# EDIpack/EDIpack

Hardware: AMD Instinct MI355X
Metric: Lanczos H*v iterations/sec, largest (Nup,Ndw) sector (higher is better)
Workload: dtype f64

## Files before the change

### edipack_amd/csrc/edigpu_apply.hip

```cpp
#include <algorithm>
#include <cmath>
#include <string>

#include "dev_mem.hpp"
#include "host_ib.hpp"
#include "kernels.hpp"

namespace edigpu {

int ensure_workspace(edigpu_sector* s) {
  const int64_t len = s->nloc * (s->is_complex ? 2 : 1);
  if (s->d_vin && s->ws_len == len) return 0;
  dev_free_all(s->d_vin, s->d_vout, s->d_tmp, s->d_partial, s->d_scal);
  const size_t n = (size_t)std::max<int64_t>(std::max(std::max(len, s->blk_len), s->ib ? s->ib->len : 0), 1);
  EDIGPU_HIP(hipMalloc((void**)&s->d_vin, n * sizeof(double)));
  EDIGPU_HIP(hipMalloc((void**)&s->d_vout, n * sizeof(double)));
  EDIGPU_HIP(hipMalloc((void**)&s->d_tmp, n * sizeof(double)));
  if (s->ib && s->ib->ps != s->ib->dim_dw * kIbPanel) {
    EDIGPU_HIP(hipMemset(s->d_vin, 0, n * sizeof(double)));
    EDIGPU_HIP(hipMemset(s->d_vout, 0, n * sizeof(double)));
    EDIGPU_HIP(hipMemset(s->d_tmp, 0, n * sizeof(double)));
  }
  s->partial_cap = std::max<int64_t>(kMaxPartials, 3 * ((s->nloc + 255) / 256) + 64);
  EDIGPU_HIP(hipMalloc((void**)&s->d_partial, (size_t)s->partial_cap * sizeof(double)));
  s->ws_len = len;
  return 0;
}

static int apply_eph_operator(const edigpu_sector* s, const double* v, double* hv, int w, hipStream_t st) {
  if (!s->sub_a) return 0;
  const int64_t n = s->dim_el * w;
  for (int jph = 0; jph <= s->nph; jph++) {
    if (apply_any(s->sub_a, v + jph * n, v + jph * n, s->d_cz, 3, st)) return 1;
    double* up = jph < s->nph ? hv + (jph + 1) * n : nullptr;
    double* dn = jph > 0 ? hv + (jph - 1) * n : nullptr;
    if (launch_eph_scatter(n, s->d_cz, up, sqrt((double)(jph + 1)), dn, sqrt((double)jph), st)) return 1;
  }
  return 0;
}

int apply_any(edigpu_sector* s, const double* v_local, const double* v_full, double* hv,
              int phase, hipStream_t st) {
  if (s->kind == kCmplxNormal) {
    if (phase != 3) {
      set_error("complex normal-mode sectors are single-shard: use the fused product");
      return 1;
    }
    if (s->sub_d) return apply_any(s->sub_d, v_full, v_full, hv, 3, st);
    const int64_t n = s->dim;
    double *xr = s->d_cz, *xi = xr + n, *yr = xi + n, *yi = yr + n, *t1 = yi + n, *t2 = t1 + n;
    if (launch_deinterleave(n, v_full, xr, xi, st)) return 1;
    if (apply_any(s->sub_s, xr, xr, yr, 3, st) || apply_any(s->sub_s, xi, xi, yi, 3, st)) return 1;
    if (s->sub_a && (apply_any(s->sub_a, xi, xi, t1, 3, st) || apply_any(s->sub_a, xr, xr, t2, 3, st))) return 1;
    return launch_combine_interleave(n, yr, yi, s->sub_a ? t1 : nullptr, s->sub_a ? t2 : nullptr, hv, st);
  }
  if (s->kind == kNormal && s->has_phonons()) {
// ... 325 lines not shown
```

### edipack_amd/csrc/edigpu_internal.hpp

```cpp
#pragma once
#include <hip/hip_runtime.h>

#include <cstdint>
#include <cstdio>
#include <functional>
#include <memory>
#include <string>
#include <vector>

#include "../../include/edigpu.h"
#include "host_build.hpp"
#include "switches.hpp"

namespace edigpu {

enum SectorKind : int { kNormal = 0, kFlat = 1, kDirect = 2, kOrbs = 3, kCmplxNormal = 4 };

void set_error(const std::string& msg);
#pragma GCC visibility push(hidden)
bool have_error();
int current_device();
int ensure_device(int* count_out = nullptr);
#pragma GCC visibility pop

// ... 175 lines not shown
  hipStream_t stream = nullptr;
  int64_t dim = 0, nloc = 0, row_first = 0;
  int64_t dim_up = 0, dim_dw = 0, dw_first = 0, dw_count = 0;
  double* d_hd = nullptr;
  edigpu::DevEll up_ell;
  edigpu::DevCsr dw;
  int dw_maxrow = 0;
  edigpu::DevCsr nd;
  int has_nd = 0;
  edigpu::HostCsr h_up, h_dw;
  int rows_per_block = 1;
  int factored = 0;
  int fac_nimp = 0, fac_nterms = 0;
  double* d_eux = nullptr;
  double* d_ed = nullptr;
  uint8_t* d_impd = nullptr;
  double* d_ndcoef = nullptr;
  uint32_t* d_jup = nullptr;
  edigpu_sector* sub_s = nullptr;
  edigpu_sector* sub_a = nullptr;
  edigpu_sector* sub_d = nullptr;
  double* d_cz = nullptr;
  int panel_mode = 0;
  int tile_nchunks = 0, tile_rows = 0;
  int32_t* d_tile_chunks = nullptr;
  int32_t* d_tile_lbeg = nullptr;
  int tile_list_cap = 0;
  int4* d_tl_meta = nullptr;
  int32_t* d_tl_col = nullptr;
  double* d_tl_val = nullptr;
  int tl_has_nd = 0;
  int blk_shift = 0;
  int blk_tail_balance = 1;
  int64_t blk_ps = 0, blk_len = 0;
  int4* d_bl_meta = nullptr;
  int blk_rows = 0;
  int blk_list_cap = 0;
  int32_t* d_bl_lend = nullptr;
  uint32_t* d_bl_ent = nullptr;
  double* d_bl_wtab = nullptr;
  bool lz_blocked = false;
  int64_t lz_len = 0;
  edigpu::IbDev* ib = nullptr;
  int row_split = 1;
  int col_halo = 0;
  uint32_t* d_jdw = nullptr;
  int32_t* d_mx_rowptr = nullptr;
  int32_t* d_mx_col = nullptr;
  double* d_mx_val = nullptr;
  int nph = 0;
  int64_t dim_el = 0;
  double w0_ph = 0.0, a_ph = 0.0;
  double* d_gu = nullptr;
  double* d_gd = nullptr;
  int64_t nd_nnz = 0;
  std::vector<double> h_hd;
  edigpu::HostCsr h_nd;
  bool lazy_export = false;
  edigpu_model model;
  int sec_a = 0, sec_b = 0;
  bool jz = false;
  bool built_by_library = false;
  bool from_model() const { return built_by_library; }
  bool is_normal_family() const { return kind == edigpu::kNormal || kind == edigpu::kCmplxNormal; }
  bool is_flat_family() const { return kind == edigpu::kFlat || kind == edigpu::kDirect; }
  bool has_phonons() const { return nph > 0; }
// ... 80 lines not shown
```

### edipack_amd/csrc/edigpu_setup.hip

```cpp
#include <algorithm>
#include <cstddef>
#include <memory>

#include "dev_mem.hpp"
#include "host_ib.hpp"
#include "host_pack.hpp"
#include "host_sb.hpp"
#include "kernels.hpp"

namespace edigpu {

static const int4* as_int4(const std::vector<HostInt4>& v) {
  static_assert(sizeof(HostInt4) == sizeof(int4) && offsetof(HostInt4, x) == offsetof(int4, x) &&
                    offsetof(HostInt4, y) == offsetof(int4, y) && offsetof(HostInt4, z) == offsetof(int4, z) &&
                    offsetof(HostInt4, w) == offsetof(int4, w),
                "HostInt4 is uploaded as int4");
  return reinterpret_cast<const int4*>(v.data());
}

static int upload_csr(DevCsr& d, int64_t nrow, const int64_t* rowptr, const int32_t* col,
                      const double* val, int cplx) {
  d = DevCsr();
  d.nrow = nrow;
  d.nnz = rowptr ? rowptr[nrow] : 0;
// ... 423 lines not shown
  if (s->factored && built && built->norb > 0 && dw_first == 0 && dw_count == dim_dw) {
    const int64_t min_rows = sw.ib_min;
    bool pairs = false;
    for (int sp = 0; sp < 2 && !pairs; sp++) {
      const std::vector<double>& a = built->ob_a[sp];
      const int ns = built->ns;
      if ((int)a.size() == ns * ns)
        for (int p = built->norb; p < ns && !pairs; p++)
          for (int q = p + 1; q < ns; q++)
            if (a[(size_t)p * ns + q] != 0.0) {
              pairs = true;
              break;
            }
    }
    const bool pairs_ok = !pairs || min_rows == 0 || sw.ib_pairs;
    const bool short_rows = dim_up * 8 < sw.ib_min_row_bytes();
    if (sw.ib && pairs_ok && s->nloc >= min_rows && (!short_rows || sw.posrows) && !sw.lanczos_unfused && setup_ib(s, *built))
      return 1;
    if (s->ib && short_rows && !s->ib->pr.on) {
      free_ib(s->ib);
      delete s->ib;
      s->ib = nullptr;
    }
  }
  if (!s->ib && s->factored && built && dw_first == 0 && dw_count == dim_dw && s->rows_per_block >= 1 && s->row_split == 1 &&
      dim_dw <= 65535 && dim_up >= 64) {
    const bool on = sw.blocked;
    const int64_t min_rows = sw.blocked_min;
    const int shift = sw.blocked_shift();
    const HostFactored& f = built->fac;
    if (on && shift == 7 && s->nloc >= min_rows && s->panel_mode == 2 && (f.nterms == 0 || s->tl_has_nd)) {
      s->blk_shift = 7;
      s->blk_tail_balance = sw.tile_balance;
      s->blk_rows = s->tile_rows;
      s->blk_ps = dim_dw << 7;
      s->blk_len = ((dim_up + 127) >> 7) * s->blk_ps;
    } else if (on && shift && shift < 7 && s->nloc >= min_rows && f.nterms <= 16) {
      const HostBlockLists b = build_block_lists(dw, f, dim_dw, shift, sw.blocked_lds_kb);
      if (b.fits) {
        s->blk_list_cap = b.list_cap;
        if (dev_upload(&s->d_bl_lend, b.lend.data(), b.lend.size()) || dev_upload(&s->d_bl_meta, as_int4(b.meta), b.meta.size()) ||
            dev_upload(&s->d_bl_ent, b.ent.data(), b.ent.size()) || dev_upload(&s->d_bl_wtab, b.wtab.data(), b.wtab.size()))
          return 1;
        s->blk_shift = shift;
        s->blk_rows = b.rows;
        s->blk_ps = dim_dw << shift;
        s->blk_len = ((dim_up + ((int64_t)1 << shift) - 1) >> shift) * s->blk_ps;
      }
    }
  }
  return finish_handle(s);
}

int setup_flat(edigpu_sector* s, int64_t nrow_local, int64_t ncol_global, int64_t row_first,
               const int64_t* rowptr, const int32_t* col, const double* val, int cplx) {
  s->kind = kFlat;
  s->is_complex = cplx;
  s->device = current_device();
  s->dim = ncol_global;
  s->nloc = nrow_local;
  s->row_first = row_first;
  const int w = cplx ? 2 : 1;
  const int64_t lo = row_first, hi = row_first + nrow_local;
  std::vector<int64_t> rpl((size_t)nrow_local + 1, 0), rpn((size_t)nrow_local + 1, 0);
  for (int64_t i = 0; i < nrow_local; i++) {
    int64_t nl = 0;
// ... 199 lines not shown
```

### edipack_amd/csrc/hooks/image_hooks.hip

```cpp
#include <algorithm>
#include <climits>

#include "../dev_mem.hpp"
#include "../host_pack.hpp"
#include "../kernels.hpp"
#include "../tile_map.hpp"

using namespace edigpu;

extern "C" {

int edigpu_tile_task_map(int32_t npanels, int32_t blocks_per_panel, int32_t balanced, int32_t* grid, int32_t* np,
                         int32_t* panel, int32_t* chunk, int32_t* pos) {
  if (npanels < 1 || blocks_per_panel < 1 || !grid || !np ||
      ((int64_t)npanels + 7) / 8 * 8 * (int64_t)blocks_per_panel > INT32_MAX) {
    set_error("edigpu_tile_task_map: bad argument");
    return 1;
  }
  const TileMap m = plan_tile_map(npanels, blocks_per_panel, balanced != 0);
  *grid = m.grid;
  *np = m.np;
  for (int wg = 0; wg < m.grid; wg++) {
    int pn, ch, ps;
    if (!tile_task_of(m, npanels, blocks_per_panel, wg, pn, ch, ps)) pn = -1;
    if (panel) panel[wg] = pn;
    if (chunk) chunk[wg] = ch;
    if (pos) pos[wg] = ps;
  }
  return 0;
}

int edigpu_ell16_images(int64_t nrow, const int64_t* rowptr, const int32_t* col, const double* val, int64_t* info,
                        uint32_t* pk16, uint32_t* pk16o, int64_t* owned_col) {
  if (nrow < 1 || !rowptr || !info || (rowptr[nrow] > 0 && (!col || !val))) {
    set_error("edigpu_ell16_images: bad argument");
    return 1;
  }
  HostCsr a;
  a.nrow = a.ncol = nrow;
  a.rowptr.assign(rowptr, rowptr + nrow + 1);
  a.col.assign(col, col + rowptr[nrow]);
  a.val.assign(val, val + rowptr[nrow]);
  const HostEll h = encode_ell(a, true, true, true);
  info[0] = h.width;
  info[1] = h.pitch;
  info[2] = h.pitch16o;
  info[3] = (int64_t)h.pk16.size();
  info[4] = (int64_t)h.pk16o.size();
  if (pk16) std::copy(h.pk16.begin(), h.pk16.end(), pk16);
  if (pk16o) std::copy(h.pk16o.begin(), h.pk16o.end(), pk16o);
  if (owned_col)
    for (int64_t pos = 0; pos < h.pitch16o; pos++) owned_col[pos] = ell16_owned_col(pos);
// ... 30 lines not shown
```

### edipack_amd/csrc/kernels_normal.hip

```cpp
#include <cstdlib>
#include <string>
#include <type_traits>

#include "kernels.hpp"
#include "normal_args.hpp"

namespace edigpu {



constexpr int kE = 4;

template <bool VEC>
__device__ inline void load4(const double* __restrict__ base, int64_t i0, const bool* ok, double* out, int64_t dB = 2) {
  if (VEC) {
    const double2 a = ok[0] ? *reinterpret_cast<const double2*>(base + i0) : make_double2(0.0, 0.0);
    const double2 b = ok[2] ? *reinterpret_cast<const double2*>(base + i0 + dB) : make_double2(0.0, 0.0);
    out[0] = a.x;
    out[1] = a.y;
    out[2] = b.x;
    out[3] = b.y;
  } else {
#pragma unroll
    for (int e = 0; e < kE; e++) out[e] = ok[e] ? base[i0 + e] : 0.0;
// ... 520 lines not shown
  a.ell_coef = s->up_ell.coef;
  a.ell_col = s->up_ell.col;
  a.ell_val = s->up_ell.val;
  a.ell_w = s->up_ell.width;
  a.ell_typed = s->up_ell.typed;
  a.ell_pitch = s->up_ell.pitch;
  a.ell_pitch16 = s->up_ell.pitch16;
  a.dw_rowptr = s->dw.rowptr32;
  a.dw_col = s->dw.col;
  a.dw_val = s->dw.val;
  a.dw_maxrow = s->dw_maxrow;
  a.nd_rp32 = s->nd.rowptr32;
  a.nd_rp64 = s->nd.wide ? s->nd.rowptr64 : nullptr;
  a.nd_col = s->nd.col;
  a.nd_val = s->nd.val;
  a.has_nd = s->has_nd;
  a.nterms = s->factored ? s->fac_nterms : 0;
  a.nd_coef = s->d_ndcoef;
  a.jup = s->d_jup;
  a.jdw = s->d_jdw;
  a.panel_mode = s->panel_mode;
  a.tile_nchunks = s->tile_nchunks;
  a.tile_rows = s->tile_rows;
  a.tile_chunks = s->d_tile_chunks;
  a.tile_lbeg = s->d_tile_lbeg;
  a.tile_list_cap = s->tile_list_cap;
  a.tl_meta = s->d_tl_meta;
  a.tl_col = s->d_tl_col;
  a.tl_val = s->d_tl_val;
  a.tl_has_nd = s->tl_has_nd;
  a.blk_shift = 0;
  a.blk_ps = 0;
  a.blk_tail_balance = s->blk_tail_balance;
  a.bl_meta = s->d_bl_meta;
  a.blk_rows = s->blk_rows;
  a.blk_list_cap = s->blk_list_cap;
  a.bl_lend = s->d_bl_lend;
  a.bl_ent = s->d_bl_ent;
  a.bl_wtab = s->d_bl_wtab;
  a.mx_rowptr = s->d_mx_rowptr;
  a.mx_col = s->d_mx_col;
  a.mx_val = s->d_mx_val;
  a.scal = nullptr;
  a.partial = nullptr;
  a.xout = nullptr;
  a.partial_cap = 0;
  a.lz_counter = nullptr;
  a.lz_nlanc = 0;
  a.lz_len = 0;
  a.split_first = 0;
  a.split_count = s->dim_up;
}

int launch_normal(const edigpu_sector* s, const double* v_local, const double* v_full, double* hv,
                  int phase, hipStream_t st) {
  NormalArgs a;
  fill_args(s, a);
  if (s->dw_count == 0) return 0;
  const bool fac = s->factored != 0;
  const bool sell_nd = !fac && s->has_nd && s->nd.sell;
  const bool csr_nd = !fac && s->has_nd && !sell_nd;
  const bool fac_nd = fac && a.nterms > 0 && s->d_mx_rowptr != nullptr;
  if (phase == 1) return launch_rows(s, a, v_local, v_full, hv, 1, st);
  if (phase == 3) {
    if (launch_rows(s, a, v_local, v_full, hv, csr_nd ? 5 : 1, st)) return 1;
    if (launch_dw_panels(a, s->sw, true, fac_nd, v_full, hv, st)) return 1;
// ... 128 lines not shown
```

### edipack_amd/csrc/kernels_panel.hip

```cpp
#include <algorithm>
#include <cstdio>
#include <cstdlib>
#include <vector>

#include "lz_finalize.hpp"
#include "normal_args.hpp"
#include "tile_map.hpp"

namespace edigpu {

struct PanelArgs {
  int npanels, width, blocks_per_panel, rows_per_block;
  int64_t col_first, ncol, stride;
  int halo;
  int tile_rows;
  int list_cap;
  TileMap map;
};

constexpr int kPanelNT = 512;
constexpr int kMaxNdTerms = 16;

template <bool DO_DW, bool DO_ND, bool ALPHA, bool COLS = false>
__global__ void __launch_bounds__(kPanelNT)
// ... 307 lines not shown
      qsum += __shfl_down(qsum, off, 64);
      nsum += __shfl_down(nsum, off, 64);
    }
    if (lane == 0) {
      red[wave] = asum;
      red[kPanelNT / 64 + wave] = qsum;
      red[2 * (kPanelNT / 64) + wave] = nsum;
    }
    __syncthreads();
    double t = 0.0, q = 0.0, n = 0.0;
    if (threadIdx.x == 0) {
#pragma unroll
      for (int i = 0; i < kPanelNT / 64; i++) {
        t += red[i];
        q += red[kPanelNT / 64 + i];
        n += red[2 * (kPanelNT / 64) + i];
      }
      if (!a.lz_counter) {
        a.partial[blockIdx.x] = t;
        a.partial[gridDim.x + blockIdx.x] = q;
        a.partial[2 * gridDim.x + blockIdx.x] = n;
      }
    }
    if (a.lz_counter)
      lz_finalize_if_last<kPanelNT>(a.lz_counter, a.partial, t, q, n, v_full, hv, a.lz_len, const_cast<double*>(a.scal),
                                    a.lz_nlanc, lzsh);
  }
}

constexpr int kTileSeg = 64;
constexpr int kTileRowsPerWave = 4;
constexpr int kTileMaxRows = kTileRowsPerWave * 16;
constexpr int kTileBatch = 4;

template <int NT, bool DO_ND, bool ALPHA, bool EDGE, bool BLK = false>
__global__ void __launch_bounds__(NT)
    normal_dw_tile_kernel(NormalArgs a, PanelArgs p, const double* __restrict__ v_full, double* __restrict__ hv) {
  __shared__ double red[3 * (NT / 64)];
  extern __shared__ double2 tile[];
  double* lval = reinterpret_cast<double*>(tile + (size_t)p.tile_rows * kTileSeg);
  int32_t* lcol = reinterpret_cast<int32_t*>(lval + p.list_cap);
  int4* lmeta = reinterpret_cast<int4*>(lcol + p.list_cap);
  uint32_t* ju2 = reinterpret_cast<uint32_t*>(lmeta + p.tile_rows);
  const int x = blockIdx.x & 7, slot = blockIdx.x >> 3, nslots = gridDim.x >> 3;
  int bpanel = 0, bchunk = 0, ppos = blockIdx.x;
  const int np = BLK ? p.map.np : (int)gridDim.x;
  const bool has_task = !BLK || tile_task_of(p.map, p.npanels, p.blocks_per_panel, blockIdx.x, bpanel, bchunk, ppos);
  if (ALPHA && BLK && (int)blockIdx.x >= p.map.wg_tail && bpanel == p.map.panel_tail && threadIdx.x < 24) {
    const int xx = threadIdx.x & 7;
    if (p.map.panel_tail + xx >= p.npanels) a.partial[(threadIdx.x >> 3) * np + ppos + xx] = 0.0;
  }
  if (ALPHA && a.scal[SC_STOP] != 0.0) {
    if (threadIdx.x == 0) {
      a.partial[ppos] = 0.0;
      a.partial[np + ppos] = 0.0;
      a.partial[2 * np + ppos] = 0.0;
    }
    return;
  }
  double asum = 0.0, qsum = 0.0, nsum = 0.0;
  const double sg = ALPHA ? a.scal[SC_ALPHA] : 0.0;
  const int lane = threadIdx.x & 63;
  const int wave = __builtin_amdgcn_readfirstlane(threadIdx.x >> 6);
  constexpr int NW = NT / 64;
  const int64_t DimUp = a.dim_up;
  int cur_panel = -1;
  for (int task = slot, it = 0;; task += nslots, it++) {
    if (BLK && (it > 0 || !has_task)) break;
    const int panel = BLK ? bpanel : (task / p.blocks_per_panel) * 8 + x;
    if (panel >= p.npanels) break;
    const int chunk = BLK ? bchunk : task % p.blocks_per_panel;
    const int rb = a.tile_chunks[chunk], nrows = a.tile_chunks[chunk + 1] - rb;
    const int lb = a.tile_lbeg[chunk], ln = a.tile_lbeg[chunk + 1] - lb;
    const int64_t pbase = (int64_t)panel * p.width;
    const int64_t RS = BLK ? 128 : DimUp;
    const double* __restrict__ vb = BLK ? v_full + (int64_t)panel * a.blk_ps : v_full;
    double* __restrict__ hb = BLK ? hv + (int64_t)panel * a.blk_ps : hv;
    auto col_of = [&](int l, bool& okl, bool& pairl) -> int64_t {
      const int64_t cl = pbase + 2 * l;
      okl = 2 * l < p.width && cl < DimUp;
      const int64_t ccl = okl ? cl : (EDGE ? DimUp - 1 : DimUp - 2);
      pairl = !EDGE || ccl + 1 < DimUp;
      return ccl;
    };
    bool ok, pair;
    int64_t cc = col_of(lane, ok, pair);
    int64_t c = pbase + 2 * lane;
    if (BLK) {
      cc = c = 2 * lane;
      ok = pair = true;
    }
    auto ld2 = [&](const double* q) -> double2 {
      if (!EDGE) return *reinterpret_cast<const double2*>(q);
      if (pair) {
        const d2u t = *reinterpret_cast<const d2u*>(q);
        return make_double2(t.x, t.y);
      }
      return make_double2(q[0], 0.0);
    };
    auto st2 = [&](double* q, double2 t) {
      if (!EDGE) {
        *reinterpret_cast<double2*>(q) = t;
      } else if (pair) {
        d2u u;
        u.x = t.x;
        u.y = t.y;
        *reinterpret_cast<d2u*>(q) = u;
      } else {
        q[0] = t.x;
      }
    };
    const int64_t g0 = a.dw_first + rb;
    double2 acc[kTileRowsPerWave];
    {
      double2 own[kTileRowsPerWave];
#pragma unroll
      for (int j = 0; j < kTileRowsPerWave; j++) {
        const int r = wave + j * NW;
        const int rr = r < nrows ? r : nrows - 1;
        acc[j] = ld2(&hb[(int64_t)(rb + rr) * RS + cc]);
      }
#pragma unroll
      for (int j = 0; j < kTileRowsPerWave; j++) {
        const int r = wave + j * NW;
        const int rr = r < nrows ? r : nrows - 1;
        own[j] = ld2(&vb[(g0 + rr) * RS + cc]);
      }
      for (int i = threadIdx.x; i < ln; i += NT) {
        lcol[i] = a.tl_col[lb + i];
        lval[i] = a.tl_val[lb + i];
      }
      if ((int)threadIdx.x < nrows) {
        int4 m = a.tl_meta[rb + threadIdx.x];
        m.x -= lb;
        lmeta[threadIdx.x] = m;
      }
#pragma unroll
      for (int j = 0; j < kTileRowsPerWave; j++) {
        const int r = wave + j * NW;
        const int rr = r < nrows ? r : nrows - 1;
        tile[rr * kTileSeg + lane] = own[j];
      }
    }
    if (DO_ND && panel != cur_panel) {
      auto encode = [&](uint32_t jt) -> uint32_t {
        if (jt == 0xFFFFFFFFu) return jt;
        const int64_t rel = (int64_t)(jt & 0x7FFFFFFFu) - pbase;
        if (rel >= 0 && rel < p.width) return (jt & 0x80000000u) | (uint32_t)rel;
        return (jt & 0x80000000u) | 0x40000000u | (jt & 0x3FFFFFFFu);
      };
      for (int i = threadIdx.x; i < 2 * a.nterms * 64; i += NT) {
        const int t2 = i >> 6, l = i & 63;
        bool okl, pairl;
        const int64_t ccl = col_of(l, okl, pairl);
        const int64_t src = (int64_t)(t2 >> 1) * DimUp + ccl;
        if (BLK) {
          const int64_t cb = pbase + 2 * l + (t2 & 1);
          ju2[i] = cb < DimUp ? encode(a.jup[(int64_t)(t2 >> 1) * DimUp + cb]) : 0xFFFFFFFFu;
          continue;
        }
        ju2[i] = (t2 & 1) ? (pairl ? encode(a.jup[src + 1]) : 0xFFFFFFFFu) : encode(a.jup[src]);
      }
      cur_panel = panel;
    }
    __syncthreads();
    auto row_sum = [&](int r, double2 s) -> double2 {
      const int4 m = lmeta[r];
      const int mb = __builtin_amdgcn_readfirstlane(m.x), ni = __builtin_amdgcn_readfirstlane(m.y),
                no = __builtin_amdgcn_readfirstlane(m.z), nn = __builtin_amdgcn_readfirstlane(m.w);
      const int ob = mb + ni, of = ob + (no & ~(kTileBatch - 1)), oe = ob + ((no + kTileBatch - 1) & ~(kTileBatch - 1));
      for (int jb = ob; jb < of; jb += kTileBatch) {
        const int4 cw = *reinterpret_cast<const int4*>(lcol + jb);
        const double2 wa = *reinterpret_cast<const double2*>(lval + jb);
        const double2 wb = *reinterpret_cast<const double2*>(lval + jb + 2);
        const double2 y0 = ld2(&vb[(int64_t)__builtin_amdgcn_readfirstlane(cw.x) * RS + cc]);
        const double2 y1 = ld2(&vb[(int64_t)__builtin_amdgcn_readfirstlane(cw.y) * RS + cc]);
        const double2 y2 = ld2(&vb[(int64_t)__builtin_amdgcn_readfirstlane(cw.z) * RS + cc]);
        const double2 y3 = ld2(&vb[(int64_t)__builtin_amdgcn_readfirstlane(cw.w) * RS + cc]);
        s.x += wa.x * y0.x;
        s.y += wa.x * y0.y;
        s.x += wa.y * y1.x;
        s.y += wa.y * y1.y;
        s.x += wb.x * y2.x;
        s.y += wb.x * y2.y;
        s.x += wb.y * y3.x;
        s.y += wb.y * y3.y;
      }
      if (const int rem = no & (kTileBatch - 1)) {
        const int4 cw = *reinterpret_cast<const int4*>(lcol + of);
        const double2 wa = *reinterpret_cast<const double2*>(lval + of);
// ... 52 lines not shown
          const bool v0 = j0 != 0xFFFFFFFFu, v1 = j1 != 0xFFFFFFFFu;
          const double w0 = v0 ? ((j0 >> 31) ? -w : w) : 0.0, w1 = v1 ? ((j1 >> 31) ? -w : w) : 0.0;
          double p0, p1;
          if (prow >= g0 && prow < g0 + nrows) {
            const double* trow = reinterpret_cast<const double*>(tile + (int)(prow - g0) * kTileSeg);
            p0 = trow[j0 & 127u];
            p1 = trow[j1 & 127u];
          } else {
            const double2 y = ld2(&vb[prow * RS + cc]);
            const int l0 = (int)((j0 >> 1) & 63u), l1 = (int)((j1 >> 1) & 63u);
            const double s0x = __shfl(y.x, l0, 64), s0y = __shfl(y.y, l0, 64);
            const double s1x = __shfl(y.x, l1, 64), s1y = __shfl(y.y, l1, 64);
            p0 = (j0 & 1u) ? s0y : s0x;
            p1 = (j1 & 1u) ? s1y : s1x;
          }
          auto edge = [&](uint32_t jw) -> double {
            const int64_t jc = (int64_t)(jw & 0x3FFFFFFFu);
            return BLK ? v_full[(jc >> 7) * a.blk_ps + prow * 128 + (jc & 127)] : v_full[prow * DimUp + jc];
          };
          if (v0 && (j0 & 0x40000000u)) p0 = edge(j0);
          if (v1 && (j1 & 0x40000000u)) p1 = edge(j1);
          s.x += w0 * p0;
          s.y += w1 * p1;
        }
      }
      return s;
    };
#pragma unroll
    for (int j = 0; j < kTileRowsPerWave; j++) {
      const int r = wave + j * NW;
      if (r < nrows) {
        acc[j] = row_sum(r, acc[j]);
        if (ok) {
          st2(&hb[(int64_t)(rb + r) * RS + c], acc[j]);
          if (ALPHA) {
            const double2 o = tile[r * kTileSeg + lane];
            const double dx = acc[j].x - sg * o.x, dy = acc[j].y - sg * o.y;
            asum += o.x * acc[j].x + o.y * acc[j].y;
            qsum += dx * dx + dy * dy;
            nsum += o.x * o.x + o.y * o.y;
          }
        }
      }
    }
    __syncthreads();
  }
  if (ALPHA) {
#pragma unroll
    for (int off = 32; off > 0; off >>= 1) {
      asum += __shfl_down(asum, off, 64);
      qsum += __shfl_down(qsum, off, 64);
      nsum += __shfl_down(nsum, off, 64);
    }
    if (lane == 0) {
      red[wave] = asum;
      red[NT / 64 + wave] = qsum;
      red[2 * (NT / 64) + wave] = nsum;
    }
    __syncthreads();
    double t = 0.0, q = 0.0, n = 0.0;
    if (threadIdx.x == 0) {
#pragma unroll
      for (int i = 0; i < NT / 64; i++) {
        t += red[i];
        q += red[NT / 64 + i];
        n += red[2 * (NT / 64) + i];
      }
// ... 221 lines not shown
    if (lane == 0) {
      red[wave] = asum;
      red[NW + wave] = qsum;
      red[2 * NW + wave] = nsum;
    }
    __syncthreads();
    double t = 0.0, q = 0.0, n = 0.0;
    if (threadIdx.x == 0) {
#pragma unroll
      for (int i = 0; i < NW; i++) {
        t += red[i];
        q += red[NW + i];
        n += red[2 * NW + i];
      }
      if (!a.lz_counter) {
        a.partial[blockIdx.x] = t;
        a.partial[gridDim.x + blockIdx.x] = q;
        a.partial[2 * gridDim.x + blockIdx.x] = n;
      }
    }
    if (a.lz_counter)
      lz_finalize_if_last<kBlkNT>(a.lz_counter, a.partial, t, q, n, v, hv, a.lz_len, const_cast<double*>(a.scal), a.lz_nlanc,
                                  lzsh);
  }
}

static int launch_dw_blocked_tiles(const NormalArgs& a, bool do_nd, const double* v, double* hv, hipStream_t st, bool alpha,
                                   int* nblocks) {
  if (!a.tile_chunks || !a.tl_meta || a.tile_rows > kTileMaxRows || (do_nd && !a.tl_has_nd) || a.dw_first != 0 ||
      a.dw_count != a.dim_dw) {
    set_error("launch_dw_blocked: 128-column panels need the tiled sweep's row lists");
    return 1;
  }
  PanelArgs p;
  p.width = 128;
  p.npanels = (int)((a.dim_up + 127) / 128);
  p.col_first = 0;
  p.ncol = a.dim_up;
  p.stride = a.dim_up;
  p.halo = 0;
  p.rows_per_block = 0;
  p.tile_rows = a.tile_rows;
  p.blocks_per_panel = a.tile_nchunks;
  p.list_cap = a.tile_list_cap;
  const int panel_groups = (p.npanels + 7) / 8;
  const int64_t np = (int64_t)panel_groups * p.blocks_per_panel * 8;
  if (np > INT32_MAX || (alpha && 3 * np > a.partial_cap)) {
    set_error("launch_dw_blocked: partial buffer too small for this grid");
    return 1;
  }
  p.map = plan_tile_map(p.npanels, p.blocks_per_panel, a.blk_tail_balance != 0 && !a.lz_counter);
  const int g = p.map.grid;
  if (nblocks) *nblocks = p.map.np;
  size_t lds = (size_t)p.tile_rows * kTileSeg * sizeof(double2) + (size_t)p.list_cap * (sizeof(double) + sizeof(int32_t)) +
               (size_t)p.tile_rows * sizeof(int4) + (do_nd ? (size_t)2 * a.nterms * 64 * sizeof(uint32_t) : 0);
  if (alpha) lds = std::max<size_t>(lds, 3 * 1024 * sizeof(double) + 16);
  const bool big = p.tile_rows > kTileRowsPerWave * (kPanelNT / 64);
#define EDIGPU_LAUNCH_BT(NTV, ND, AL)                                                   \
  do {                                                                                  \
    auto kern = normal_dw_tile_kernel<NTV, ND, AL, false, true>;                        \
    if (ensure_dynamic_lds((const void*)kern, lds)) return 1;                           \
    hipLaunchKernelGGL(kern, dim3((unsigned)g), dim3(NTV), lds, st, a, p, v, hv);       \
  } while (0)
#define EDIGPU_LAUNCH_BT2(ND, AL)          \
  do {                                     \
    if (big)                               \
      EDIGPU_LAUNCH_BT(1024, ND, AL);      \
    else                                   \
      EDIGPU_LAUNCH_BT(kPanelNT, ND, AL);  \
  } while (0)
  if (do_nd && alpha)
    EDIGPU_LAUNCH_BT2(true, true);
  else if (do_nd)
    EDIGPU_LAUNCH_BT2(true, false);
  else if (alpha)
    EDIGPU_LAUNCH_BT2(false, true);
  else
    EDIGPU_LAUNCH_BT2(false, false);
#undef EDIGPU_LAUNCH_BT2
#undef EDIGPU_LAUNCH_BT
  EDIGPU_HIP(hipGetLastError());
  return 0;
}

int launch_dw_blocked(const NormalArgs& a, const Switches& sw, bool do_nd, const double* v, double* hv, hipStream_t st, bool alpha,
                      int* nblocks) {
  if (a.blk_shift == 7) return launch_dw_blocked_tiles(a, do_nd, v, hv, st, alpha, nblocks);
  if (a.blk_shift < 4 || a.blk_shift > 6 || a.blk_rows < 32 || !a.bl_meta || !a.bl_ent || !a.bl_wtab || !a.bl_lend || a.blk_list_cap < 4 || a.dw_first != 0 ||
      a.dw_count != a.dim_dw) {
    set_error("launch_dw_blocked: the sector has no panel-major image");
    return 1;
  }
  if (do_nd && a.nterms > kMaxNdTerms) {
// ... 227 lines not shown
```

### edipack_amd/csrc/normal_args.hpp

```cpp
#pragma once
#include <cstdint>

#include "kernels.hpp"

namespace edigpu {

struct NormalArgs {
  int64_t dim_up, dim_dw, dw_first, dw_count;
  const double* hd;
  const double* eux;
  const double* ed;
  const uint8_t* impd;
  const uint32_t* ell_pk;
  const double* ell_coef;
  const uint32_t* ell_pk16;
  const int32_t* ell_col;
  const double* ell_val;
  int ell_w;
  int ell_typed;
  int64_t split_first, split_count;
  int64_t ell_pitch;
  int64_t ell_pitch16;
  const int32_t* dw_rowptr;
  const int32_t* dw_col;
  const double* dw_val;
  const int32_t* nd_rp32;
  const int64_t* nd_rp64;
  const int32_t* nd_col;
  const double* nd_val;
  int dw_maxrow;
  int has_nd;
  int nterms;
  const double* nd_coef;
  const uint32_t* jup;
  const uint32_t* jdw;
  const double* scal;
  double* partial;
  double* xout;
  int64_t partial_cap;
  unsigned int* lz_counter;
  int lz_nlanc;
  int64_t lz_len;
  int panel_mode;
  int tile_nchunks, tile_rows;
  const int32_t* tile_chunks;
  const int32_t* tile_lbeg;
  int tile_list_cap;
  const int4* tl_meta;
  const int32_t* tl_col;
  const double* tl_val;
  int tl_has_nd;
  int blk_shift;
  int blk_tail_balance;
  int64_t blk_ps;
  const int4* bl_meta;
  const uint32_t* bl_ent;
  int blk_rows;
  int blk_list_cap;
  const int32_t* bl_lend;
  const double* bl_wtab;
  const int32_t* mx_rowptr;
  const int32_t* mx_col;
  const double* mx_val;
};

int launch_dw_panels(const NormalArgs& a, const Switches& sw, bool do_dw, bool do_nd, const double* v_full, double* hv,
                     hipStream_t st, bool alpha = false, int* nblocks = nullptr);

int launch_dw_blocked(const NormalArgs& a, const Switches& sw, bool do_nd, const double* v, double* hv, hipStream_t st, bool alpha,
                      int* nblocks);

int launch_dw_panel_cols(const NormalArgs& a, const Switches& sw, bool do_nd, int64_t col_first, int64_t ncol, int64_t stride, int halo,
                         const double* w, double* hv, hipStream_t st);

}
```

### edipack_amd/csrc/switches.hpp

```cpp
#pragma once
#include <cstdint>
#include <limits>
#include <optional>

namespace edigpu {

enum class SwitchRule {
  Present,
  FirstIsOne,
  OnUnlessZero,
  OffUnlessNonzero,
  Int,
  Int64,
  IntOrUnset,
  Int64OrUnset,
  DoubleOrUnset,
};
enum class SwitchMoment { SetUp, Comm, Loop };

struct SwitchRow {
  const char* name;
  SwitchRule rule;
  int64_t dflt, lo, hi;
  SwitchMoment moment;
  const char* what;
};
const SwitchRow* switch_table(int* nrows);

constexpr int64_t kSwAny = std::numeric_limits<int64_t>::max();
using OptInt = std::optional<int>;
using OptInt64 = std::optional<int64_t>;
using OptDouble = std::optional<double>;

#define EDIGPU_SETUP_SWITCHES(X)                                                                                                            \
                                                                                                         \
  X(ell16, bool, "EDIGPU_ELL16", OnUnlessZero, 1, 0, 1, "0: no 16-bit LDS image of Hup beside the packed one")                              \
  X(ell_untyped, bool, "EDIGPU_ELL_UNTYPED", Present, 0, 0, 1, "Hup as plain ELL (column, value), not the packed typed image")            \
  X(csr_nosell, bool, "EDIGPU_CSR_NOSELL", Present, 0, 0, 1, "stored sectors stay CSR: no SELL-64 image")                                  \
  X(csr_unpacked, bool, "EDIGPU_CSR_UNPACKED", Present, 0, 0, 1, "SELL-64 image with explicit values, not the value dictionary")          \
  X(normal_explicit, bool, "EDIGPU_NORMAL_EXPLICIT", FirstIsOne, 0, 0, 1, "normal mode: explicit diagonal and Hnd, not the factored tables") \
  X(handover_factor, bool, "EDIGPU_HANDOVER_FACTOR", OnUnlessZero, 1, 0, 1, "0: handed-over arrays are not searched for the factored form") \
  X(nd_in_rows, bool, "EDIGPU_ND_IN_ROWS", FirstIsOne, 0, 0, 1, "explicit Hnd as CSR inside the row kernel, not as its own SELL pass")     \
  X(nd_no_merge, bool, "EDIGPU_ND_NO_MERGE", Present, 0, 0, 1, "factored Hnd terms of equal partner maps are not merged")                  \
  X(cmplx_fourproducts, bool, "EDIGPU_CMPLX_FOURPRODUCTS", FirstIsOne, 0, 0, 1, "complex normal mode as four real products, not the doubled real sector") \
  X(flat_hostbuild, bool, "EDIGPU_FLAT_HOSTBUILD", FirstIsOne, 0, 0, 1, "stored superc / nonsu2 image built on the host, not on the device") \
  X(direct_nosort, bool, "EDIGPU_DIRECT_NOSORT", Present, 0, 0, 1, "on-the-fly terms keep the builder's order")                            \
  X(direct_termorder, bool, "EDIGPU_DIRECT_TERMORDER", Present, 0, 0, 1, "on-the-fly kernel walks all terms, no per-workgroup compaction") \
  X(direct_wgs, int, "EDIGPU_DIRECT_WGS", Int, 2, -kSwAny, kSwAny, "on-the-fly kernel: persistent workgroups per CU")                      \
                                                                      \
  X(rows_td, OptInt, "EDIGPU_ROWS_TD", IntOrUnset, 0, 0, 0, "rows per workgroup of the LDS row kernel (1, 2, 4, 8); unset: from the row length") \
  X(row_split, OptInt, "EDIGPU_ROW_SPLIT", IntOrUnset, 0, 0, 0, "column parts long rows are staged in (0: never); unset: as many as the LDS needs") \
  X(panel_vec2, bool, "EDIGPU_PANEL_VEC2", OnUnlessZero, 1, 0, 1, "0: no two-column panel sweep")                                          \
  X(panel_vec2_min, int64_t, "EDIGPU_PANEL_VEC2_MIN", Int64, (int64_t)1 << 21, -kSwAny, kSwAny, "smallest sector (rows) of the two-column and tiled sweeps") \
  X(panel_tile, bool, "EDIGPU_PANEL_TILE", OnUnlessZero, 1, 0, 1, "0: no LDS-tiled panel sweep")                                           \
  X(tile_rows, int, "EDIGPU_TILE_ROWS", Int, 32, 8, 64, "rows of a chunk of the tiled sweep")                                               \
  X(tile_balance, bool, "EDIGPU_TILE_BALANCE", OnUnlessZero, 1, 0, 1, "0: padded grid of the tiled sweep, last panel group not spread over the XCDs") \
  X(tile_persist, bool, "EDIGPU_TILE_PERSIST", OffUnlessNonzero, 0, 0, 1, "tiled sweep as a persistent grid")                              \
  X(panel_w, OptInt, "EDIGPU_PANEL_W", IntOrUnset, 0, 0, 0, "widest panel (columns); unset or out of range: 64, two-column sweep 128")      \
  X(panel_bpp, OptInt, "EDIGPU_PANEL_BPP", IntOrUnset, 0, 0, 0, "workgroups per panel; unset: 128, two-column sweep 256")                   \
  X(blocked, bool, "EDIGPU_BLOCKED", OnUnlessZero, 1, 0, 1, "0: the Lanczos loop keeps the natural vector layout")                         \
  X(blocked_min, int64_t, "EDIGPU_BLOCKED_MIN", Int64, (int64_t)1 << 21, -kSwAny, kSwAny, "smallest sector (rows) of the panel-major loop") \
  X(blocked_w, int, "EDIGPU_BLOCKED_W", Int, 128, -kSwAny, kSwAny, "panel width of that loop: 128 (tiled sweep), 64 / 32 / 16 (narrow-panel sweep); else none") \
  X(blocked_lds_kb, int64_t, "EDIGPU_BLOCKED_LDS_KB", Int64, 32, -kSwAny, kSwAny, "KiB of staged segments per block of the narrow-panel sweep") \
  X(blocked_wgs, int, "EDIGPU_BLOCKED_WGS", Int, 8, -kSwAny, kSwAny, "narrow-panel sweep: workgroups per CU (1 .. 8, else 8)")             \
                                                                                                                  \
  X(ib, bool, "EDIGPU_IB", OnUnlessZero, 1, 0, 1, "0: no impurity-block image")                                                            \
  X(ib_min, int64_t, "EDIGPU_IB_MIN", Int64, (int64_t)1 << 21, -kSwAny, kSwAny, "smallest sector (elements) that gets it; 0 also lifts the row and pair gates") \
  X(ib_minrow, OptInt64, "EDIGPU_IB_MINROW", Int64OrUnset, 0, 0, 0, "shortest row (bytes) on its rows kernels; unset: 40960, or 0 when EDIGPU_IB_MIN=0") \
  X(ib_rows, int, "EDIGPU_IB_ROWS", Int, 480, 4, 480, "rows of a staged chunk of its columns kernel")                                       \
  X(ib_pairs, bool, "EDIGPU_IB_PAIRS", FirstIsOne, 0, 0, 1, "replica / general baths take the image too")                                  \
  X(ib_split, OptInt, "EDIGPU_IB_SPLIT", IntOrUnset, 0, 0, 0, "rows staged in halves: non-zero always, 0 never; unset: rows longer than the LDS") \
  X(ib_nsub, int, "EDIGPU_IB_NSUB", Int, 1, 1, 8, "workgroups per chunk of the columns kernel")                                            \
  X(ib_pspad, int, "EDIGPU_IB_PSPAD", Int, 0, 0, kSwAny, "doubles between two panels (rounded down to even)")                              \
  X(ib_nt, int, "EDIGPU_IB_NT", Int, 0, -kSwAny, kSwAny, "threads per workgroup of the rows kernel; 0: the best that fits")                \
  X(ib_cols2, OptInt, "EDIGPU_IB_COLS2", IntOrUnset, 0, 0, 0, "pipelined columns kernel: non-zero on, 0 off; unset: panels above 2 MiB")   \
  X(ib_verbose, bool, "EDIGPU_IB_VERBOSE", Present, 0, 0, 1, "say on stderr why a sector gets no image")                                   \
  X(posrows, bool, "EDIGPU_POSROWS", OffUnlessNonzero, 0, 0, 1, "short rows: the generic LDS row kernel in position order beside the block columns kernel") \
                                                                                                      \
  X(sb, bool, "EDIGPU_SB", OnUnlessZero, 1, 0, 1, "0: the impurity-block kernels, no local-block tables")                                  \
  X(sb_split, bool, "EDIGPU_SB_SPLIT", OffUnlessNonzero, 0, 0, 1, "local-block rows kernel on rows staged in halves")                      \
  X(sb_amode, bool, "EDIGPU_SB_AMODE", OffUnlessNonzero, 0, 0, 1, "per-orbital walk where the bath allows it")                             \
  X(sb_cw, int, "EDIGPU_SB_CW", Int, 0, -kSwAny, kSwAny, "columns kernel: 1 = one column per lane, 512 threads; else two, 256 threads")    \
  X(sb_nt, int, "EDIGPU_SB_NT", Int, 0, -kSwAny, kSwAny, "threads per workgroup of the rows kernel; 0: the first geometry that fits")      \
  X(sb_nbt, int, "EDIGPU_SB_NBT", Int, 0, -kSwAny, kSwAny, "blocks per thread of the rows kernel; 0: likewise")                            \
  X(sb_stamp, bool, "EDIGPU_SB_STAMP", Present, 0, 0, 1, "print cycle stamps of the rows kernel per launch")                               \
  X(sb_verbose, bool, "EDIGPU_SB_VERBOSE", Present, 0, 0, 1, "say on stderr which tables a sector gets, or why none")                      \
                                                                                                             \
  X(lanczos_unfused, bool, "EDIGPU_LANCZOS_UNFUSED", Present, 0, 0, 1, "literal recurrence: product, then the vector kernels")             \
  X(lanczos_inkernel_finalize, bool, "EDIGPU_LANCZOS_INKERNEL_FINALIZE", OffUnlessNonzero, 0, 0, 1, "the sweep's last workgroup finalizes the step") \
// ... 39 lines not shown
```

### edipack_amd/csrc/tile_map.hpp

```cpp
#pragma once

#if defined(__HIPCC__)
#define EDIGPU_TILE_HD __host__ __device__
#else
#define EDIGPU_TILE_HD
#endif

namespace edigpu {

struct TileMap {
  int grid;
  int np;
  int wg_tail;
  int panel_tail;
  int q, r;
};

inline TileMap plan_tile_map(int npanels, int blocks_per_panel, bool balance) {
  TileMap m;
  const int t = npanels % 8;
  m.np = (npanels + 7) / 8 * blocks_per_panel * 8;
  m.grid = m.wg_tail = m.np;
  m.panel_tail = npanels;
  m.q = m.r = 0;
  if (balance && t != 0) {
    m.panel_tail = npanels - t;
    m.wg_tail = m.panel_tail * blocks_per_panel;
    m.q = t * blocks_per_panel / 8;
    m.r = t * blocks_per_panel % 8;
    m.grid = m.wg_tail + t * blocks_per_panel;
  }
  return m;
}

EDIGPU_TILE_HD inline bool tile_task_of(const TileMap& m, int npanels, int blocks_per_panel, int wg, int& panel, int& chunk,
                                        int& pos) {
  const int x = wg & 7;
  if (wg >= m.wg_tail) {
    const int i = x * m.q + (x < m.r ? x : m.r) + ((wg - m.wg_tail) >> 3);
    panel = m.panel_tail + i / blocks_per_panel;
    chunk = i % blocks_per_panel;
    pos = ((panel >> 3) * blocks_per_panel + chunk) * 8 + (panel & 7);
    return true;
  }
  panel = ((wg >> 3) / blocks_per_panel) * 8 + x;
  chunk = (wg >> 3) % blocks_per_panel;
  pos = wg;
  return panel < npanels;
}

}
```

Measured before the change: 7513.

## Add opt-in half-panel tiled sweep splitting 128-column panels into 64-column passes

Adds an EDIGPU_TILE_HALF switch, off by default. When set, the blocked tiled sweep processes each 128-column panel as two 64-column units, which doubles the workgroups per panel. The tile task map, partial-buffer sizing and tail-balance logic are generalized to handle these sub-panel units. Blocked-layout stores now go through a raw buffer store with a bounded resource descriptor, and this path is taken whenever BLK is set, including the default. The aim is more parallelism and occupancy on large sectors, at the cost of half the lanes idling in half mode and extra indexing complexity.

```diff
diff --git a/edipack_amd/csrc/edigpu_apply.hip b/edipack_amd/csrc/edigpu_apply.hip
--- a/edipack_amd/csrc/edigpu_apply.hip
+++ b/edipack_amd/csrc/edigpu_apply.hip
@@ -22,6 +22,8 @@
     EDIGPU_HIP(hipMemset(s->d_tmp, 0, n * sizeof(double)));
   }
   s->partial_cap = std::max<int64_t>(kMaxPartials, 3 * ((s->nloc + 255) / 256) + 64);
+  if (s->blk_shift == 7)
+    s->partial_cap = std::max<int64_t>(s->partial_cap, 3 * (((s->dim_up + 127) / 128 + 7) / 8 * 8) * (s->blk_tile_half ? 2 : 1) * s->tile_nchunks);
   EDIGPU_HIP(hipMalloc((void**)&s->d_partial, (size_t)s->partial_cap * sizeof(double)));
   s->ws_len = len;
   return 0;
diff --git a/edipack_amd/csrc/edigpu_internal.hpp b/edipack_amd/csrc/edigpu_internal.hpp
--- a/edipack_amd/csrc/edigpu_internal.hpp
+++ b/edipack_amd/csrc/edigpu_internal.hpp
@@ -231,6 +231,7 @@
   int tl_has_nd = 0;
   int blk_shift = 0;
   int blk_tail_balance = 1;
+  int blk_tile_half = 0;
   int64_t blk_ps = 0, blk_len = 0;
   int4* d_bl_meta = nullptr;
   int blk_rows = 0;
diff --git a/edipack_amd/csrc/edigpu_setup.hip b/edipack_amd/csrc/edigpu_setup.hip
--- a/edipack_amd/csrc/edigpu_setup.hip
+++ b/edipack_amd/csrc/edigpu_setup.hip
@@ -479,6 +479,7 @@
     if (on && shift == 7 && s->nloc >= min_rows && s->panel_mode == 2 && (f.nterms == 0 || s->tl_has_nd)) {
       s->blk_shift = 7;
       s->blk_tail_balance = sw.tile_balance;
+      s->blk_tile_half = sw.tile_half && !sw.lanczos_inkernel_finalize;
       s->blk_rows = s->tile_rows;
       s->blk_ps = dim_dw << 7;
       s->blk_len = ((dim_up + 127) >> 7) * s->blk_ps;
diff --git a/edipack_amd/csrc/hooks/image_hooks.hip b/edipack_amd/csrc/hooks/image_hooks.hip
--- a/edipack_amd/csrc/hooks/image_hooks.hip
+++ b/edipack_amd/csrc/hooks/image_hooks.hip
@@ -12,12 +12,13 @@
 
 int edigpu_tile_task_map(int32_t npanels, int32_t blocks_per_panel, int32_t balanced, int32_t* grid, int32_t* np,
                          int32_t* panel, int32_t* chunk, int32_t* pos) {
-  if (npanels < 1 || blocks_per_panel < 1 || !grid || !np ||
-      ((int64_t)npanels + 7) / 8 * 8 * (int64_t)blocks_per_panel > INT32_MAX) {
+  const int per = (balanced & 2) ? 2 : 1;
+  if (npanels < 1 || blocks_per_panel < 1 || !grid || !np || balanced < 0 || balanced > 3 || npanels % per != 0 ||
+      ((int64_t)npanels / per + 7) / 8 * 8 * (int64_t)per * blocks_per_panel > INT32_MAX) {
     set_error("edigpu_tile_task_map: bad argument");
     return 1;
   }
-  const TileMap m = plan_tile_map(npanels, blocks_per_panel, balanced != 0);
+  const TileMap m = plan_tile_map(npanels, blocks_per_panel, (balanced & 1) != 0, per);
   *grid = m.grid;
   *np = m.np;
   for (int wg = 0; wg < m.grid; wg++) {
diff --git a/edipack_amd/csrc/kernels_normal.hip b/edipack_amd/csrc/kernels_normal.hip
--- a/edipack_amd/csrc/kernels_normal.hip
+++ b/edipack_amd/csrc/kernels_normal.hip
@@ -576,6 +576,7 @@
   a.blk_shift = 0;
   a.blk_ps = 0;
   a.blk_tail_balance = s->blk_tail_balance;
+  a.blk_tile_half = s->blk_tile_half;
   a.bl_meta = s->d_bl_meta;
   a.blk_rows = s->blk_rows;
   a.blk_list_cap = s->blk_list_cap;
diff --git a/edipack_amd/csrc/kernels_panel.hip b/edipack_amd/csrc/kernels_panel.hip
--- a/edipack_amd/csrc/kernels_panel.hip
+++ b/edipack_amd/csrc/kernels_panel.hip
@@ -363,8 +363,10 @@
 constexpr int kTileRowsPerWave = 4;
 constexpr int kTileMaxRows = kTileRowsPerWave * 16;
 constexpr int kTileBatch = 4;
-
-template <int NT, bool DO_ND, bool ALPHA, bool EDGE, bool BLK = false>
+typedef double tile_d2 __attribute__((ext_vector_type(2)));
+typedef unsigned int tile_u4 __attribute__((ext_vector_type(4)));
+
+template <int NT, bool DO_ND, bool ALPHA, bool EDGE, bool BLK = false, bool HALF = false>
 __global__ void __launch_bounds__(NT)
     normal_dw_tile_kernel(NormalArgs a, PanelArgs p, const double* __restrict__ v_full, double* __restrict__ hv) {
   __shared__ double red[3 * (NT / 64)];
@@ -377,9 +379,9 @@
   int bpanel = 0, bchunk = 0, ppos = blockIdx.x;
   const int np = BLK ? p.map.np : (int)gridDim.x;
   const bool has_task = !BLK || tile_task_of(p.map, p.npanels, p.blocks_per_panel, blockIdx.x, bpanel, bchunk, ppos);
-  if (ALPHA && BLK && (int)blockIdx.x >= p.map.wg_tail && bpanel == p.map.panel_tail && threadIdx.x < 24) {
+  if (ALPHA && BLK && (int)blockIdx.x >= p.map.wg_tail && bpanel / p.map.per_panel == p.map.panel_tail && threadIdx.x < 24) {
     const int xx = threadIdx.x & 7;
-    if (p.map.panel_tail + xx >= p.npanels) a.partial[(threadIdx.x >> 3) * np + ppos + xx] = 0.0;
+    if (p.map.panel_tail + xx >= p.npanels / p.map.per_panel) a.partial[(threadIdx.x >> 3) * np + ppos + xx] = 0.0;
   }
   if (ALPHA && a.scal[SC_STOP] != 0.0) {
     if (threadIdx.x == 0) {
@@ -405,8 +407,9 @@
     const int lb = a.tile_lbeg[chunk], ln = a.tile_lbeg[chunk + 1] - lb;
     const int64_t pbase = (int64_t)panel * p.width;
     const int64_t RS = BLK ? 128 : DimUp;
-    const double* __restrict__ vb = BLK ? v_full + (int64_t)panel * a.blk_ps : v_full;
-    double* __restrict__ hb = BLK ? hv + (int64_t)panel * a.blk_ps : hv;
+    const double* __restrict__ vb = BLK ? v_full + (int64_t)(HALF ? panel >> 1 : panel) * a.blk_ps : v_full;
+    double* __restrict__ hb = BLK ? hv + (int64_t)(HALF ? panel >> 1 : panel) * a.blk_ps : hv;
+    const auto qrsrc = __builtin_amdgcn_make_buffer_rsrc(hb, 0, BLK ? (int)(a.dim_dw * 128 * sizeof(double)) : 0, 0x00020000);
     auto col_of = [&](int l, bool& okl, bool& pairl) -> int64_t {
       const int64_t cl = pbase + 2 * l;
       okl = 2 * l < p.width && cl < DimUp;
@@ -418,8 +421,9 @@
     int64_t cc = col_of(lane, ok, pair);
     int64_t c = pbase + 2 * lane;
     if (BLK) {
-      cc = c = 2 * lane;
-      ok = pair = true;
+      cc = c = HALF ? 64 * (panel & 1) + 2 * (lane & 31) : 2 * lane;
+      pair = true;
+      ok = !HALF || lane < 32;
     }
     auto ld2 = [&](const double* q) -> double2 {
       if (!EDGE) return *reinterpret_cast<const double2*>(q);
@@ -486,7 +490,7 @@
         const int64_t ccl = col_of(l, okl, pairl);
         const int64_t src = (int64_t)(t2 >> 1) * DimUp + ccl;
         if (BLK) {
-          const int64_t cb = pbase + 2 * l + (t2 & 1);
+          const int64_t cb = pbase + 2 * (HALF ? l & 31 : l) + (t2 & 1);
           ju2[i] = cb < DimUp ? encode(a.jup[(int64_t)(t2 >> 1) * DimUp + cb]) : 0xFFFFFFFFu;
           continue;
         }
@@ -605,7 +609,15 @@
       if (r < nrows) {
         acc[j] = row_sum(r, acc[j]);
         if (ok) {
-          st2(&hb[(int64_t)(rb + r) * RS + c], acc[j]);
+          if (BLK) {
+            tile_d2 t;
+            t.x = acc[j].x;
+            t.y = acc[j].y;
+            __builtin_amdgcn_raw_buffer_store_b128(__builtin_bit_cast(tile_u4, t), qrsrc,
+                                                   (int)(((rb + r) * 128 + (int)c) * sizeof(double)), 0, 16);
+          } else {
+            st2(&hb[(int64_t)(rb + r) * RS + c], acc[j]);
+          }
           if (ALPHA) {
             const double2 o = tile[r * kTileSeg + lane];
             const double dx = acc[j].x - sg * o.x, dy = acc[j].y - sg * o.y;
@@ -893,9 +905,11 @@
     set_error("launch_dw_blocked: 128-column panels need the tiled sweep's row lists");
     return 1;
   }
+  const bool half = a.blk_tile_half != 0 && !a.lz_counter;
+  const int per = half ? 2 : 1;
   PanelArgs p;
-  p.width = 128;
-  p.npanels = (int)((a.dim_up + 127) / 128);
+  p.width = 128 / per;
+  p.npanels = (int)((a.dim_up + 127) / 128) * per;
   p.col_first = 0;
   p.ncol = a.dim_up;
   p.stride = a.dim_up;
@@ -904,13 +918,13 @@
   p.tile_rows = a.tile_rows;
   p.blocks_per_panel = a.tile_nchunks;
   p.list_cap = a.tile_list_cap;
-  const int panel_groups = (p.npanels + 7) / 8;
-  const int64_t np = (int64_t)panel_groups * p.blocks_per_panel * 8;
+  const int panel_groups = (p.npanels / per + 7) / 8;
+  const int64_t np = (int64_t)panel_groups * per * p.blocks_per_panel * 8;
   if (np > INT32_MAX || (alpha && 3 * np > a.partial_cap)) {
     set_error("launch_dw_blocked: partial buffer too small for this grid");
     return 1;
   }
-  p.map = plan_tile_map(p.npanels, p.blocks_per_panel, a.blk_tail_balance != 0 && !a.lz_counter);
+  p.map = plan_tile_map(p.npanels, p.blocks_per_panel, a.blk_tail_balance != 0 && !a.lz_counter, per);
   const int g = p.map.grid;
   if (nblocks) *nblocks = p.map.np;
   size_t lds = (size_t)p.tile_rows * kTileSeg * sizeof(double2) + (size_t)p.list_cap * (sizeof(double) + sizeof(int32_t)) +
@@ -919,7 +933,8 @@
   const bool big = p.tile_rows > kTileRowsPerWave * (kPanelNT / 64);
 #define EDIGPU_LAUNCH_BT(NTV, ND, AL)                                                   \
   do {                                                                                  \
-    auto kern = normal_dw_tile_kernel<NTV, ND, AL, false, true>;                        \
+    auto kern = half ? normal_dw_tile_kernel<NTV, ND, AL, false, true, true>            \
+                     : normal_dw_tile_kernel<NTV, ND, AL, false, true, false>;          \
     if (ensure_dynamic_lds((const void*)kern, lds)) return 1;                           \
     hipLaunchKernelGGL(kern, dim3((unsigned)g), dim3(NTV), lds, st, a, p, v, hv);       \
   } while (0)
diff --git a/edipack_amd/csrc/normal_args.hpp b/edipack_amd/csrc/normal_args.hpp
--- a/edipack_amd/csrc/normal_args.hpp
+++ b/edipack_amd/csrc/normal_args.hpp
@@ -52,6 +52,7 @@
   int tl_has_nd;
   int blk_shift;
   int blk_tail_balance;
+  int blk_tile_half;
   int64_t blk_ps;
   const int4* bl_meta;
   const uint32_t* bl_ent;
diff --git a/edipack_amd/csrc/switches.hpp b/edipack_amd/csrc/switches.hpp
--- a/edipack_amd/csrc/switches.hpp
+++ b/edipack_amd/csrc/switches.hpp
@@ -55,6 +55,7 @@
   X(panel_tile, bool, "EDIGPU_PANEL_TILE", OnUnlessZero, 1, 0, 1, "0: no LDS-tiled panel sweep")                                           \
   X(tile_rows, int, "EDIGPU_TILE_ROWS", Int, 32, 8, 64, "rows of a chunk of the tiled sweep")                                               \
   X(tile_balance, bool, "EDIGPU_TILE_BALANCE", OnUnlessZero, 1, 0, 1, "0: padded grid of the tiled sweep, last panel group not spread over the XCDs") \
+  X(tile_half, bool, "EDIGPU_TILE_HALF", OffUnlessNonzero, 0, 0, 1, "tiled sweep on 128-column panels in half-panel passes of 64 columns") \
   X(tile_persist, bool, "EDIGPU_TILE_PERSIST", OffUnlessNonzero, 0, 0, 1, "tiled sweep as a persistent grid")                              \
   X(panel_w, OptInt, "EDIGPU_PANEL_W", IntOrUnset, 0, 0, 0, "widest panel (columns); unset or out of range: 64, two-column sweep 128")      \
   X(panel_bpp, OptInt, "EDIGPU_PANEL_BPP", IntOrUnset, 0, 0, 0, "workgroups per panel; unset: 128, two-column sweep 256")                   \
diff --git a/edipack_amd/csrc/tile_map.hpp b/edipack_amd/csrc/tile_map.hpp
--- a/edipack_amd/csrc/tile_map.hpp
+++ b/edipack_amd/csrc/tile_map.hpp
@@ -14,39 +14,44 @@
   int wg_tail;
   int panel_tail;
   int q, r;
+  int per_panel;
 };
 
-inline TileMap plan_tile_map(int npanels, int blocks_per_panel, bool balance) {
+inline TileMap plan_tile_map(int nunits, int blocks_per_panel, bool balance, int per_panel = 1) {
   TileMap m;
+  const int npanels = nunits / per_panel, T = per_panel * blocks_per_panel;
   const int t = npanels % 8;
-  m.np = (npanels + 7) / 8 * blocks_per_panel * 8;
+  m.per_panel = per_panel;
+  m.np = (npanels + 7) / 8 * T * 8;
   m.grid = m.wg_tail = m.np;
   m.panel_tail = npanels;
   m.q = m.r = 0;
   if (balance && t != 0) {
     m.panel_tail = npanels - t;
-    m.wg_tail = m.panel_tail * blocks_per_panel;
-    m.q = t * blocks_per_panel / 8;
-    m.r = t * blocks_per_panel % 8;
-    m.grid = m.wg_tail + t * blocks_per_panel;
+    m.wg_tail = m.panel_tail * T;
+    m.q = t * T / 8;
+    m.r = t * T % 8;
+    m.grid = m.wg_tail + t * T;
   }
   return m;
 }
 
-EDIGPU_TILE_HD inline bool tile_task_of(const TileMap& m, int npanels, int blocks_per_panel, int wg, int& panel, int& chunk,
+EDIGPU_TILE_HD inline bool tile_task_of(const TileMap& m, int nunits, int blocks_per_panel, int wg, int& unit, int& chunk,
                                         int& pos) {
-  const int x = wg & 7;
+  const int x = wg & 7, T = m.per_panel * blocks_per_panel;
   if (wg >= m.wg_tail) {
     const int i = x * m.q + (x < m.r ? x : m.r) + ((wg - m.wg_tail) >> 3);
-    panel = m.panel_tail + i / blocks_per_panel;
+    unit = m.panel_tail * m.per_panel + i / blocks_per_panel;
     chunk = i % blocks_per_panel;
-    pos = ((panel >> 3) * blocks_per_panel + chunk) * 8 + (panel & 7);
+    const int panel = unit / m.per_panel, half = unit % m.per_panel;
+    pos = ((panel >> 3) * T + half * blocks_per_panel + chunk) * 8 + (panel & 7);
     return true;
   }
-  panel = ((wg >> 3) / blocks_per_panel) * 8 + x;
-  chunk = (wg >> 3) % blocks_per_panel;
+  const int panel = ((wg >> 3) / T) * 8 + x, w = (wg >> 3) % T;
+  unit = panel * m.per_panel + w / blocks_per_panel;
+  chunk = w % blocks_per_panel;
   pos = wg;
-  return panel < npanels;
+  return unit < nunits;
 }
 
 }
```

After: 7585, median of 6. About the same (+1.0%).
